# sahaRatul/sela

Measured on AMD Instinct MI355X. Metric: Msamples/s encode+decode, 16-bit stereo 44.1kHz, 1/2/4/8 GPU; bit-exact vs CPU, higher is better.
Workload: dtype f64+int64

## Files before the change

### sela_amd/csrc/sela_encode.hip

```cpp
#include <algorithm>
#include <atomic>
#include <random>
#include <vector>

#include "sela_device.h"

namespace sela {

constexpr int kPadC = 64;
constexpr int kHalfEntries = kBlock / 4;
constexpr int kParityLen = kPadC + kHalfEntries + 64;
constexpr int kLastT0 = (kHalfEntries + 64) / 32 - 1;
constexpr int kFirstT1 = (kHalfEntries - kPadC) / 32;
constexpr int kRingHalf = 64;
constexpr int kRingLen = 2 * kRingHalf + 64;
constexpr int kRingsPerXcd = 512;
constexpr int kXcds = 8;
constexpr int kPadS = 128;
constexpr int kSBufWords = (kPadS + kBlock) / 32 * 33;
constexpr int kSmallBase = 8992;
constexpr int kBigBytes = kSmallBase + 3008;
static_assert(kResWordsCap * 4 <= kSmallBase, "packed residue words must fit the dead sample buffer");
static_assert(kSBufWords * 4 <= kSmallBase && kSmallBase % 16 == 0, "sample buffer must end below the analysis arrays");
static_assert(kBigBytes >= 2 * kParityLen * 8, "the FP64 parity arrays must fit");

struct SmallArrays {
    double ac[104];
    double k[104];
    int64_t a[104];
    int32_t q[128];
};
static_assert(sizeof(SmallArrays) + kSmallBase <= kBigBytes, "analysis arrays overflow the LDS plan");

__device__ __forceinline__ void or_bits(uint32_t* buf, uint32_t pos, uint32_t v, uint32_t nbits)
{
    const uint32_t w = pos >> 5, sh = pos & 31;
    atomicOr(&buf[w], v << sh);
    if (sh + nbits > 32)
        atomicOr(&buf[w + 1], v >> (32 - sh));
}

__device__ __forceinline__ void or_bits_both(uint32_t* buf, uint32_t pos, uint32_t v)
{
    const uint64_t wide = (uint64_t)v << (pos & 31);
    uint32_t* const w = buf + (pos >> 5);
    atomicOr(w, (uint32_t)wide);
    atomicOr(w + 1, (uint32_t)(wide >> 32));
}

__device__ __attribute__((noinline)) uint32_t put_long_codeword(uint32_t* buf, uint32_t pos, uint32_t u, uint32_t k);

__device__ __forceinline__ uint32_t put_codeword(uint32_t* buf, uint32_t pos, uint32_t u, uint32_t k)
{
    uint32_t ones = u >> k;
    const uint32_t rem = k ? (__brev(u << (32 - k))) : 0u;
    while (ones >= 32) {
        or_bits(buf, pos, 0xFFFFFFFFu, 32);
        pos += 32;
        ones -= 32;
    }
    if (ones + 1 + k <= 32) {
        or_bits(buf, pos, ((1u << ones) - 1u) | (rem << (ones + 1)), ones + 1 + k);
        return pos + ones + 1 + k;
    }
    or_bits(buf, pos, (1u << ones) - 1u, ones + 1);
    pos += ones + 1;
    if (k) {
        or_bits(buf, pos, rem, k);
        pos += k;
    }
    return pos;
}

__device__ __attribute__((noinline)) uint32_t put_long_codeword(uint32_t* buf, uint32_t pos, uint32_t u, uint32_t k)
{
    return put_codeword(buf, pos, u, k);
}

template <int V>
__device__ __forceinline__ uint64_t rice_shifted_sum(const uint32_t (&u)[V], uint32_t k, bool small, uint32_t& lane_part)
{
    if (small) {
        uint32_t part = 0;
#pragma unroll
        for (int t = 0; t < V; t++)
            part += u[t] >> k;
        asm volatile("" : "+v"(part));
        lane_part = part;
        return wave_sum_small(part);
    }
    uint64_t part = 0;
#pragma unroll
    for (int t = 0; t < V; t++)
        part += u[t] >> k;
    lane_part = (uint32_t)part;
    return wave_sum_40(part);
}

template <int V>
__device__ __forceinline__ void rice_plan(const uint32_t (&u)[V], uint32_t n, uint32_t& best_k, uint64_t& best_bits, uint32_t& lane_or, uint32_t& lane_quotients)
{
    constexpr uint32_t kLast = SELA_MAX_RICE_PARAM - 1;
    lane_or = 0;
#pragma unroll
    for (int t = 0; t < V; t++)
        lane_or |= u[t];
    const bool small = !__any((lane_or >> 20) != 0);
    uint32_t p0, pa, pb, pc;
    const uint64_t t0 = rice_shifted_sum<V>(u, 0, small, p0);
    const uint64_t mean = n ? t0 / n : 0;
    uint32_t k = mean ? 63u - (uint32_t)__clzll(mean) : 0u;
    k = k > kLast - 1 ? kLast - 1 : k;
    uint64_t ta = t0;
    pa = p0;
    if (k)
        ta = rice_shifted_sum<V>(u, k, small, pa);
    uint64_t tb = rice_shifted_sum<V>(u, k + 1, small, pb);
    if (ta - tb <= n) {
        while (k > 0) {
            uint64_t tc = t0;
            pc = p0;
            if (k != 1)
                tc = rice_shifted_sum<V>(u, k - 1, small, pc);
            if (tc - ta > n)
                break;
            k--;
            tb = ta, pb = pa;
            ta = tc, pa = pc;
        }
    } else {
        for (;;) {
            k++;
            ta = tb, pa = pb;
            if (k == kLast)
                break;
            tb = rice_shifted_sum<V>(u, k + 1, small, pb);
            if (ta - tb <= n)
                break;
        }
    }
    best_k = k;
    best_bits = ta + (uint64_t)n * (1 + k);
    lane_quotients = pa;
}

__device__ __forceinline__ double scale_sample(int32_t s)
{
    constexpr double r = 1.0 / SELA_SAMPLE_SCALE;
    const double x = (double)s;
    const double q0 = x * r;
    const double e = __builtin_fma(-SELA_SAMPLE_SCALE, q0, x);
    return __builtin_fma(e, r, q0);
}

template <int kN>
__device__ __forceinline__ void unpack_stereo(uint32_t sig, const uint32_t (&w)[kN], int32_t (&raw)[kN])
{
    if (sig == 0) {
#pragma unroll
        for (int i = 0; i < kN; i++)
            raw[i] = (int32_t)(int16_t)(w[i] & 0xFFFFu);
    } else if (sig == 1) {
#pragma unroll
        for (int i = 0; i < kN; i++)
            raw[i] = (int32_t)w[i] >> 16;
    } else {
#pragma unroll
        for (int i = 0; i < kN; i++)
            raw[i] = (int32_t)(int16_t)(w[i] & 0xFFFFu) - ((int32_t)w[i] >> 16);
    }
}

typedef double f64x2 __attribute__((ext_vector_type(2)));
struct MeanFetch {
    f64x2 e0, e1, e2, e3, o0, o1, o2, o3;
};
#define SELA_MEAN_STR2(x) #x
#define SELA_MEAN_STR(x) SELA_MEAN_STR2(x)
#define SELA_MEAN_ISSUE(F, addr, OFF, sum)                                                    \
    asm volatile("ds_read_b128 %0, %9 offset:" #OFF "+0\n\t"                                    \
                 "ds_read_b128 %4, %9 offset:" #OFF "+5120\n\t"                                 \
                 "ds_read_b128 %1, %9 offset:" #OFF "+16\n\t"                                   \
                 "ds_read_b128 %5, %9 offset:" #OFF "+5136\n\t"                                 \
                 "ds_read_b128 %2, %9 offset:" #OFF "+32\n\t"                                   \
                 "ds_read_b128 %6, %9 offset:" #OFF "+5152\n\t"                                 \
                 "ds_read_b128 %3, %9 offset:" #OFF "+48\n\t"                                   \
                 "ds_read_b128 %7, %9 offset:" #OFF "+5168"                                      \
                 : "=&v"(F.e0), "=&v"(F.e1), "=&v"(F.e2), "=&v"(F.e3), "=&v"(F.o0), "=&v"(F.o1), "=&v"(F.o2), \
                 "=&v"(F.o3), "+v"(sum)                                                         \
                 : "v"(addr)                                                                    \
                 : "memory")
static_assert(kParityLen * 8 == 5120, "SELA_MEAN_ISSUE hard-codes the E -> O distance");

__device__ __forceinline__ void mean_wait(MeanFetch& f, double& sum)
{
    asm volatile("s_waitcnt lgkmcnt(0)"
                 : "+v"(f.e0), "+v"(f.e1), "+v"(f.e2), "+v"(f.e3), "+v"(f.o0), "+v"(f.o1), "+v"(f.o2), "+v"(f.o3), "+v"(sum));
}

__device__ __forceinline__ void mean_steps(const MeanFetch& f, double& sum)
{
    sum += f.e0[0]; sum += f.o0[0]; sum += f.e0[1]; sum += f.o0[1];
    sum += f.e1[0]; sum += f.o1[0]; sum += f.e1[1]; sum += f.o1[1];
    sum += f.e2[0]; sum += f.o2[0]; sum += f.e2[1]; sum += f.o2[1];
    sum += f.e3[0]; sum += f.o3[0]; sum += f.e3[1]; sum += f.o3[1];
}

typedef int sgpr16 __attribute__((ext_vector_type(16)));
typedef double f64x8 __attribute__((ext_vector_type(8)));

struct AcFetch {
    sgpr16 c_lo, c_hi;
    f64x2 o0, o1, o2, o3;
    f64x2 e0, e1, e2, e3;
};

#define SELA_AC_ISSUE_S(F, c_ptr, S0, S1, acc_e, acc_o)                                   \
    asm volatile("s_load_dwordx16 %0, %4, " #S0 "\n\ts_load_dwordx16 %1, %4, " #S1          \
                 : "=&s"(F.c_lo), "=&s"(F.c_hi), "+v"(acc_e), "+v"(acc_o) : "s"(c_ptr) : "memory")

#define SELA_AC_ISSUE_V(F, addr_e, addr_o, Q0, Q1, Q2, Q3, Q4, Q5, Q6, Q7, Q8, acc_e, acc_o) \
    asm volatile("ds_read2_b64 %0, %11 offset0:" #Q0 " offset1:" #Q1 "\n\t"                   \
                 "ds_read2_b64 %4, %10 offset0:" #Q1 " offset1:" #Q2 "\n\t"                   \
                 "ds_read2_b64 %1, %11 offset0:" #Q2 " offset1:" #Q3 "\n\t"                   \
                 "ds_read2_b64 %5, %10 offset0:" #Q3 " offset1:" #Q4 "\n\t"                   \
                 "ds_read2_b64 %2, %11 offset0:" #Q4 " offset1:" #Q5 "\n\t"                   \
                 "ds_read2_b64 %6, %10 offset0:" #Q5 " offset1:" #Q6 "\n\t"                   \
                 "ds_read2_b64 %3, %11 offset0:" #Q6 " offset1:" #Q7 "\n\t"                   \
                 "ds_read2_b64 %7, %10 offset0:" #Q7 " offset1:" #Q8                           \
                 : "=&v"(F.o0), "=&v"(F.o1), "=&v"(F.o2), "=&v"(F.o3), "=&v"(F.e0), "=&v"(F.e1), \
                 "=&v"(F.e2), "=&v"(F.e3), "+v"(acc_e), "+v"(acc_o)                           \
                 : "v"(addr_e), "v"(addr_o)                                                   \
                 : "memory")

__device__ __forceinline__ void ac_wait(AcFetch& f, double& acc_e, double& acc_o)
{
    asm volatile("s_waitcnt lgkmcnt(0)"
                 : "+s"(f.c_lo), "+s"(f.c_hi), "+v"(f.o0), "+v"(f.o1), "+v"(f.o2), "+v"(f.o3), "+v"(f.e0), "+v"(f.e1),
                 "+v"(f.e2), "+v"(f.e3), "+v"(acc_e), "+v"(acc_o));
}

__device__ __forceinline__ void ac_step(double cj, double nw, double& A, double& B, double& acc_e, double& acc_o)
{
    acc_e += cj * A;
    acc_o += cj * B;
    B = A;
    A = nw;
}

__device__ __forceinline__ void ac_steps_head(const AcFetch& f, double& A, double& B, double& acc_e, double& acc_o)
{
    const f64x8 c = __builtin_bit_cast(f64x8, f.c_lo);
    ac_step(c[0], f.o0[0], A, B, acc_e, acc_o);
    ac_step(c[1], f.e0[0], A, B, acc_e, acc_o);
}

__device__ __forceinline__ void ac_steps_tail(const AcFetch& f, double& A, double& B, double& acc_e, double& acc_o)
{
    const f64x8 c = __builtin_bit_cast(f64x8, f.c_lo), d = __builtin_bit_cast(f64x8, f.c_hi);
    ac_step(c[2], f.o0[1], A, B, acc_e, acc_o);
    ac_step(c[3], f.e0[1], A, B, acc_e, acc_o);
    ac_step(c[4], f.o1[0], A, B, acc_e, acc_o);
    ac_step(c[5], f.e1[0], A, B, acc_e, acc_o);
    ac_step(c[6], f.o1[1], A, B, acc_e, acc_o);
    ac_step(c[7], f.e1[1], A, B, acc_e, acc_o);
    ac_step(d[0], f.o2[0], A, B, acc_e, acc_o);
    ac_step(d[1], f.e2[0], A, B, acc_e, acc_o);
    ac_step(d[2], f.o2[1], A, B, acc_e, acc_o);
    ac_step(d[3], f.e2[1], A, B, acc_e, acc_o);
    ac_step(d[4], f.o3[0], A, B, acc_e, acc_o);
    ac_step(d[5], f.e3[0], A, B, acc_e, acc_o);
    ac_step(d[6], f.o3[1], A, B, acc_e, acc_o);
    ac_step(d[7], f.e3[1], A, B, acc_e, acc_o);
}

template <int JJ>
__device__ __forceinline__ void fir_taps_f64(int j0, int order, const int32_t* s_grp, const double* a_grp,
    double (&win)[kPerLane], double (&acc)[kPerLane])
{
    const int j = j0 + JJ + 1;
    if (j > order)
        return;
    const double aj = a_grp[JJ + 1];
    win[(32 - JJ - 1) & 31] = (double)s_grp[31 - JJ];
#pragma unroll
    for (int t = 0; t < kPerLane; t++)
        acc[t] = __builtin_fma(aj, win[(t - JJ - 1) & 31], acc[t]);
    __builtin_amdgcn_sched_barrier(0);
    if constexpr (JJ < 31)
        fir_taps_f64<JJ + 1>(j0, order, s_grp, a_grp, win, acc);
}
__device__ __forceinline__ const int32_t* fir_group_window(const int32_t* sT, int lane, int j0)
{
    const int e = kPadS + 32 * lane - j0 - 32;
    return sT + e + (e >> 5);
}
__device__ __forceinline__ const double* fir_group_coefs(const double* a_f, int j0)
{
    uint32_t at = (uint32_t)(uintptr_t)(const __attribute__((address_space(3))) double*)(a_f + j0);
    asm volatile("" : "+v"(at));
    return (const double*)(const __attribute__((address_space(3))) double*)(uintptr_t)at;
}

__device__ __attribute__((noinline)) void fir_plain(int order, int lane, const int32_t* sT, const int64_t* a, uint32_t* pred_out)
{
#pragma unroll 1
    for (int t = 0; t < kPerLane; t++) {
        uint64_t sum = (uint64_t)1 << (SELA_Q_SHIFT - 1);
#pragma unroll 1
        for (int j = 1; j <= order; j++) {
            const int e = kPadS + 32 * lane + t - j;
            sum += (uint64_t)a[j] * (uint64_t)(int64_t)sT[e + (e >> 5)];
        }
        pred_out[t * 64 + lane] = (uint32_t)(int32_t)((int64_t)sum >> SELA_Q_SHIFT);
    }
}

constexpr uint32_t kFuseSpinLimit = 1u << 18;
constexpr uint32_t kFuseNapLimit = 600000;
constexpr uint32_t kMeanWaitSpins = 24;

__device__ __forceinline__ void block_of(uint32_t e, uint32_t n_sig, uint32_t& frame, uint32_t& sig)
{
// ... 714 lines not shown
        asm volatile("s_waitcnt vmcnt(0)\n\ts_dcache_inv" ::: "memory");

        double A = E[-lane];
        double B = 0.0;
        uint32_t addr_e = (uint32_t)(uintptr_t)(__attribute__((address_space(3))) double*)(E - lane);
        uint32_t addr_o = (uint32_t)(uintptr_t)(__attribute__((address_space(3))) double*)(O - lane);
        const double* c_ptr = ring;
        AcFetch f0, f1;
        asm volatile("" : "+v"(A));
        SELA_AC_ISSUE_S(f0, c_ptr, 0, 64, acc_e, acc_o);
        SELA_AC_ISSUE_V(f0, addr_e, addr_o, 0, 1, 2, 3, 4, 5, 6, 7, 8, acc_e, acc_o);
        constexpr int kSwitch = kBlock / 2 / kRingHalf;
        const bool falling = !kFused && n_workers == 0 && fa.priorities != 0;
#pragma unroll 1
        for (int k = 0; k < kBlock / kRingHalf; k++) {
            if (falling && k == 0)
                __builtin_amdgcn_s_setprio(2);
            if (falling && k == kSwitch)
                __builtin_amdgcn_s_setprio(1);
            if (k == kSwitch) {
                wave_sync();
#pragma unroll
                for (int t = kFirstT1; t < kPerLane; t++)
                    mine1[half + 32 * t] = scale_sample(s[t]) - mean;
                wave_sync();
                addr_e -= kHalfEntries * 8;
                addr_o -= kHalfEntries * 8;
            }
            if (k >= 1 && k + 1 < kBlock / kRingHalf)
                store_chunk(k + 1, k >= kSwitch ? mine1 : mine);
#pragma unroll 1
            for (int it = 0; it < kRingHalf / 32; it++) {
                if (it == kRingHalf / 32 - 1)
                    asm volatile("s_waitcnt vmcnt(0)\n\ts_dcache_inv" ::: "memory");
                ac_wait(f0, acc_e, acc_o);
                SELA_AC_ISSUE_S(f1, c_ptr, 128, 192, acc_e, acc_o);
                ac_steps_head(f0, A, B, acc_e, acc_o);
                SELA_AC_ISSUE_V(f1, addr_e, addr_o, 8, 9, 10, 11, 12, 13, 14, 15, 16, acc_e, acc_o);
                ac_steps_tail(f0, A, B, acc_e, acc_o);
                ac_wait(f1, acc_e, acc_o);
                SELA_AC_ISSUE_S(f0, c_ptr, 256, 320, acc_e, acc_o);
                ac_steps_head(f1, A, B, acc_e, acc_o);
                SELA_AC_ISSUE_V(f0, addr_e, addr_o, 16, 17, 18, 19, 20, 21, 22, 23, 24, acc_e, acc_o);
                ac_steps_tail(f1, A, B, acc_e, acc_o);
                c_ptr += 32;
                addr_e += 128;
                addr_o += 128;
            }
            if (k & 1)
                c_ptr = ring;
        }
        ac_wait(f0, acc_e, acc_o);
        if (lane == 0)
            atomicExch(pool + slot, 0u);
    }
    wave_sync();

    SELA_STAMP(4);
    {
        const double ac0 = read_first_lane(acc_e);
        if (lane <= 50) {
            sm->ac[2 * lane] = lane == 0 ? 1.0 : acc_e / ac0;
            sm->ac[2 * lane + 1] = acc_o / ac0;
        }
    }
    wave_sync();

    double k_lo = 0.0, k_hi = 0.0;
    if (!kFused && n_workers == 0 && fa.priorities != 0)
        __builtin_amdgcn_s_setprio(1);
    else
        __builtin_amdgcn_s_setprio(2);
    {
        double g0a = sm->ac[lane + 1], g1a = g0a;
        double g0b = lane < 36 ? sm->ac[lane + 65] : 0.0, g1b = g0b;
        double err = 1.0;
        double g = read_first_lane(g1a);
        double ki = -g / err;
        err += g * ki;
        sm->k[0] = ki;
        constexpr int kTwoRegs = kMaxOrder - 64 + 1;
#pragma unroll 1
        for (int i = 1; i < kTwoRegs; i++) {
            const double sa = wave_shl1(read_first_lane(g1b), g1a);
            const double sb = wave_shl1_zero(g1b);
            g1a = sa + ki * g0a;
            g0a = sa * ki + g0a;
            g1b = sb + ki * g0b;
            g0b = sb * ki + g0b;
            g = read_first_lane(g1a);
            ki = -g / err;
            err += g * ki;
            sm->k[i] = ki;
        }
#pragma unroll 1
        for (int i = kTwoRegs; i < kMaxOrder; i++) {
            const double sa = wave_shl1_zero(g1a);
            g1a = sa + ki * g0a;
            g0a = sa * ki + g0a;
            g = read_first_lane(g1a);
            ki = -g / err;
            err += g * ki;
            sm->k[i] = ki;
        }
        wave_sync();
        k_lo = sm->k[lane];
        k_hi = lane < kMaxOrder - 64 ? sm->k[lane + 64] : 0.0;
        wave_sync();
    }
    if (kMode == 3) {
        uint64_t h_ac = hash_term(sm->ac[lane], lane) ^ (lane + 64 <= kMaxOrder ? hash_term(sm->ac[lane + 64], lane + 64) : 0ull);
        uint64_t h_k = hash_term(k_lo, lane) ^ (lane < kMaxOrder - 64 ? hash_term(k_hi, lane + 64) : 0ull);
        h_ac = lanes_xor<64>(h_ac);
        h_k = lanes_xor<64>(h_k);
        if (lane == 0) {
            uint64_t* const hp = reinterpret_cast<uint64_t*>(trace) + 2 * (size_t)block_id;
            hp[0] = h_ac;
            hp[1] = h_k;
        }
    }

    {
        constexpr bool kAcInLds = true;
        uint64_t* const sizes_pub = fa.sizes_pub;
        const uint64_t sizes_tag = fa.sizes_tag;
#define SELA_TAIL_TRACE_RESIDUES fa.trace_residues
#include "sela_encode_tail.inc"
#undef SELA_TAIL_TRACE_RESIDUES
    }
    SELA_STAMP(12);
    if (kFused) {
        const uint32_t g = frame / kGroupFrames;
        const uint32_t blocks_in_group = min((uint32_t)kGroupFrames, n_frames - g * kGroupFrames) * n_sig;
        stores_done();
        uint32_t last = 0;
        if (lane == 0)
            last = group_arrive(fa.group_count + (size_t)g * kGroupCountStride, fa.tag, blocks_in_group) ? 1u : 0u;
        if (__builtin_amdgcn_readfirstlane((int)last)) {
            drop_stale_lines();
            finish_group(fa, g, lane);
        }
    }
    SELA_STAMP(13);
    if (kMode == 2 && lane == 0)
        for (int i = 0; i < 13; i++)
            phase_cycles[(size_t)block_id * 16 + i] = (uint64_t)(stamp[i + 1] - stamp[i]);
}

constexpr int kTeamMirror = 24;
constexpr int kTeamWin = 16;
constexpr int kTeamAhead = 3;
constexpr int kTeamMeanChunk = 64;

template <int P>
struct TeamPlan {
    static constexpr int B = kWave / P;
    static constexpr int G = (kMaxOrder + 1 + P - 1) / P;
    static constexpr int kChunk = P == 8 ? 16 : 64;
    static constexpr int kRing = P == 8 ? 160 : 256;
    static constexpr int kStride = P == 8 ? kRing + kTeamMirror : kRing + 48;
    static constexpr int kPer = kChunk / P;
    static constexpr int kMeanPer = kTeamMeanChunk / P;
    static constexpr int kRingBytes = B * kStride * 8;
    static constexpr int kCwBase = kBigBytes;
    static constexpr int kKStride = 104;
    static constexpr int kQBase = kSmallBase;
    static constexpr int kQStride = 104;
    static constexpr int kSchurBase = B * kKStride;
    static constexpr int kSchurStride = P == 16 ? 2 * P * G : 0;
    static constexpr int kSchurBytes = P == 16 ? (kSchurBase + B * kSchurStride) * 8 : 0;
    static constexpr int kTailBytes = kCwBase + kCoefWordsCap * 4;
    static constexpr int kLdsBytes = kRingBytes > kTailBytes ? kRingBytes : kTailBytes;
    static_assert(kSchurBytes <= kLdsBytes, "the repack areas fit the kernel's LDS");
    static_assert(G + kTeamAhead <= kTeamWin && kChunk % kTeamWin == 0 && kRing % kChunk == 0 && kStride % 32 == (P == 8 ? 24 : 16) && kStride >= kRing + kTeamMirror, "team plan");
    static_assert((G * P - 1) + kChunk + kChunk <= kRing && 2 * kTeamMeanChunk <= kRing, "the ring must hold the lags' reach, the chunk in use and the chunk being written");
    static_assert(kLdsBytes * 12 <= 160 * 1024, "twelve waves per CU");
    static_assert(B * kKStride * 8 <= kQBase && B * kKStride * 8 <= kRingBytes && B * kQStride <= 104 * 8, "k[] in the dead rings below the q store; the q store inside SmallArrays::ac");
};

template <int P>
__device__ __forceinline__ uint32_t team_first(uint32_t v)
{
    if constexpr (P == 16) {
        return (uint32_t)__builtin_amdgcn_mov_dpp((int)v, 0x150 , 0xf, 0xf, true);
    } else {
        static_assert(P == 8, "teams of 8 or 16 lanes");
        const int q = __builtin_amdgcn_mov_dpp((int)v, 0x00 , 0xf, 0xf, true);
        return (uint32_t)__builtin_amdgcn_update_dpp(q, q, 0x114 , 0xf, 0xa , false);
    }
}
template <int P>
__device__ __forceinline__ double team_first(double v)
{
    const uint64_t x = __builtin_bit_cast(uint64_t, v);
    return __builtin_bit_cast(double, ((uint64_t)team_first<P>((uint32_t)(x >> 32)) << 32) | team_first<P>((uint32_t)x));
}

template <int kPer, int kStep>
__device__ __forceinline__ void team_load_raw(const int16_t* __restrict__ fp, uint32_t channels, uint32_t sig, int first, int32_t (&raw)[kPer])
{
    if (channels == 2) {
        const uint32_t* pw = reinterpret_cast<const uint32_t*>(fp) + first;
        uint32_t w[kPer];
        if constexpr (kStep == 1 && kPer % 4 == 0) {
#pragma unroll
            for (int u = 0; u < kPer / 4; u++) {
                const uint4 v = reinterpret_cast<const uint4*>(pw)[u];
                w[4 * u] = v.x, w[4 * u + 1] = v.y, w[4 * u + 2] = v.z, w[4 * u + 3] = v.w;
            }
        } else if constexpr (kStep == 1 && kPer % 2 == 0) {
#pragma unroll
            for (int u = 0; u < kPer / 2; u++) {
                const uint2 v = reinterpret_cast<const uint2*>(pw)[u];
                w[2 * u] = v.x, w[2 * u + 1] = v.y;
            }
        } else {
#pragma unroll
            for (int u = 0; u < kPer; u++)
                w[u] = pw[u * kStep];
        }
        if constexpr (kStep == 1) {
            const uint32_t first_shift = sig == 1 ? 16u : 0u;
            const uint32_t second_mask = sig == 2 ? 0xFFFFFFFFu : 0u;
#pragma unroll
            for (int i = 0; i < kPer; i++) {
                const int32_t a = (int32_t)(w[i] << (16 - first_shift)) >> 16, b = ((int32_t)w[i] >> 16) & (int32_t)second_mask;
                raw[i] = a - b;
            }
        } else {
            unpack_stereo<kPer>(sig, w, raw);
        }
    } else {
        const int16_t* const ps = fp + (size_t)first * channels + sig;
#pragma unroll
        for (int i = 0; i < kPer; i++)
            raw[i] = ps[(uint32_t)(i * kStep) * channels];
    }
}

template <int kPer, int kStep, bool kStereo>
__device__ __forceinline__ void team_fetch(const int16_t* __restrict__ fp, uint32_t channels, uint32_t sig, int first, uint32_t (&w)[kPer])
{
    if constexpr (kStereo) {
        const uint32_t* pw = reinterpret_cast<const uint32_t*>(fp) + first;
#pragma unroll
        for (int u = 0; u < kPer; u++)
            w[u] = pw[u * kStep];
    } else {
        const int16_t* const ps = fp + (size_t)first * channels + sig;
#pragma unroll
        for (int i = 0; i < kPer; i++)
            w[i] = (uint32_t)(int32_t)ps[(uint32_t)(i * kStep) * channels];
    }
}
template <int kPer, bool kStereo>
__device__ __forceinline__ void team_unpack(uint32_t sig, const uint32_t (&w)[kPer], int32_t (&raw)[kPer])
{
    if constexpr (kStereo) {
        unpack_stereo<kPer>(sig, w, raw);
    } else {
#pragma unroll
        for (int i = 0; i < kPer; i++)
            raw[i] = (int32_t)w[i];
    }
}

template <int kPer, int kStep, bool kCentre, bool kMirror, int kRing>
__device__ __forceinline__ void team_stage(double* ring_b, int pos, const int32_t (&raw)[kPer], double mean)
{
#pragma unroll
    for (int i = 0; i < kPer; i++) {
        const double x = scale_sample(raw[i]);
        const double c = kCentre ? x - mean : x;
        ring_b[pos + i * kStep] = c;
        if (kMirror && pos + i * kStep < kTeamMirror)
            ring_b[kRing + pos + i * kStep] = c;
    }
}

template <int kN>
__device__ __forceinline__ double team_chain(const double* x, double sum)
{
    constexpr int kBatch = 8;
    static_assert(kN % (2 * kBatch) == 0, "two batches per round");
    double u[kBatch], v[kBatch];
#pragma unroll
    for (int i = 0; i < kBatch; i++)
        u[i] = x[i];
#pragma unroll
    for (int i0 = 0; i0 < kN; i0 += 2 * kBatch) {
#pragma unroll
        for (int i = 0; i < kBatch; i++)
            v[i] = x[i0 + kBatch + i];
        __builtin_amdgcn_sched_barrier(0);
#pragma unroll
        for (int i = 0; i < kBatch; i++)
            sum += u[i];
        __builtin_amdgcn_sched_barrier(0);
        if (i0 + 2 * kBatch < kN) {
#pragma unroll
            for (int i = 0; i < kBatch; i++)
                u[i] = x[i0 + 2 * kBatch + i];
        }
        __builtin_amdgcn_sched_barrier(0);
#pragma unroll
        for (int i = 0; i < kBatch; i++)
// ... 63 lines not shown
                 : "v"(addr_w), "v"(addr_m), "n"(8 * (R0 + kTeamAhead)), "v"(acc[0]), "v"(acc[G - 1])
                 : "memory");
    asm volatile("s_waitcnt lgkmcnt(6)" : "+v"(W[R0 & (kTeamWin - 1)]), "+v"(M[R0 & 3]));
    const double m = M[R0 & 3];
    constexpr int kAheadOps = 5;
#pragma unroll
    for (int g0 = 0; g0 < G; g0 += kAheadOps) {
        double t[kAheadOps];
#pragma unroll
        for (int u = 0; u < kAheadOps; u++)
            if (g0 + u < G)
                t[u] = m * W[(R0 - g0 - u) & (kTeamWin - 1)];
#pragma unroll
        for (int u = 0; u < kAheadOps; u++)
            if (g0 + u < G)
                acc[g0 + u] += t[u];
    }
    __builtin_amdgcn_sched_barrier(0);
    if constexpr (R0 < kTeamWin - 1)
        team_ac_steps<G, R0 + 1>(W, M, acc, addr_w, addr_m);
}

template <int P>
struct TeamSchur {
    static constexpr int G = TeamPlan<P>::G;
    static constexpr bool kPhased = P == 16;
    static constexpr int kFirstStage(int g) { return g >= G || !kPhased ? 1 : kMaxOrder + 1 - P * g; }
    static constexpr int kEndStage(int g) { return g == 1 || !kPhased ? kMaxOrder : kFirstStage(g - 1); }
};

template <int P, int gFrom, int gTo>
__device__ __forceinline__ void team_schur_repack(double (&g0)[TeamPlan<P>::G], double (&g1)[TeamPlan<P>::G], double* __restrict__ area, int p)
{
    double* const w = area + gFrom * p;
    const double* const r = area + gTo * p;
#pragma unroll
    for (int c = 0; c < gFrom; c++) {
        w[c] = g0[c];
        w[P * gFrom + c] = g1[c];
    }
    wave_sync();
#pragma unroll
    for (int c = 0; c < gTo; c++) {
        g0[c] = r[c];
        g1[c] = r[P * gFrom + c];
    }
    wave_sync();
}

template <int P, int g>
__device__ __forceinline__ void team_schur_phases(double (&g0)[TeamPlan<P>::G], double (&g1)[TeamPlan<P>::G], double& ki, double& err,
    bool keeper, double* __restrict__ k_b, double* __restrict__ area, int p)
{
    using S = TeamSchur<P>;
    static_assert(S::kFirstStage(g) >= 1 && S::kFirstStage(g) < S::kEndStage(g) && P * g - 1 >= kMaxOrder - S::kFirstStage(g), "a phase starts when its last column is dead");
#pragma unroll 1
    for (int i = S::kFirstStage(g); i < S::kEndStage(g); i++) {
        const double crossing = wave_shl1_zero(g1[0]);
#pragma unroll
        for (int r = 0; r < g; r++) {
            const double sa = r + 1 < g ? g1[r + 1] : crossing;
            g1[r] = sa + ki * g0[r];
            g0[r] = sa * ki + g0[r];
        }
        const double first = team_first<P>(g1[0]);
        ki = -first / err;
        err += first * ki;
        if (keeper)
            k_b[i] = ki;
    }
    if constexpr (S::kPhased && g > 1) {
        team_schur_repack<P, g, g - 1>(g0, g1, area, p);
        team_schur_phases<P, g - 1>(g0, g1, ki, err, keeper, k_b, area, p);
    }
}

template <int kMode, int P>
__global__ __launch_bounds__(64) __attribute__((amdgpu_waves_per_eu(3, 3))) void k_encode_teams(
    const int16_t* __restrict__ pcm, uint32_t n_frames, uint32_t channels, uint32_t n_sig, BlockMeta* __restrict__ meta,
    uint32_t* __restrict__ slots, sela_hip_trace* __restrict__ trace, int force_plain_fir, uint64_t* __restrict__ phase_cycles,
    uint64_t* __restrict__ sizes_pub, uint64_t sizes_tag, uint32_t team_priorities)
{
    using Plan = TeamPlan<P>;
    constexpr int B = Plan::B, G = Plan::G, kPer = Plan::kPer, kMeanPer = Plan::kMeanPer, kChunk = Plan::kChunk, kRing = Plan::kRing;
    constexpr bool kTrace = kMode == 1;
    constexpr bool kFused = false;
    constexpr int kStep = P == 16 ? P : 1;
    __shared__ __attribute__((aligned(32))) unsigned char lds[Plan::kLdsBytes];
    unsigned char* const big = lds;
    uint32_t* const cw_buf = reinterpret_cast<uint32_t*>(lds + Plan::kCwBase);

    const int lane0 = threadIdx.x;
    const int b = lane0 / P, p = lane0 % P;
    const uint32_t wq = blockIdx.x % 8, wv = blockIdx.x / 8;
    const uint32_t sig = wv % n_sig;
    const uint32_t frame0 = ((wv / n_sig) * 8 + wq) * B;
    constexpr uint32_t frame_stride = 1;
    if (frame0 >= n_frames)
        return;
    const bool team_live = frame0 + (uint32_t)b * frame_stride < n_frames;
    const uint32_t my_frame = team_live ? frame0 + (uint32_t)b * frame_stride : frame0;
    const int16_t* const fp = pcm + (size_t)my_frame * kBlock * channels;
    double* const ring_b = reinterpret_cast<double*>(lds) + b * Plan::kStride;
    double* const k_b = reinterpret_cast<double*>(lds) + b * Plan::kKStride;
    long long wave_stamp[5];
    if (kMode == 2)
        wave_stamp[0] = clock64();

    double mean;
    if constexpr (P == 16) {
        static_assert(kStep == P, "lane p holds samples p, p + 16, .. of a chunk");
        set_wave_priority((int)(team_priorities & 0xFF));
        const double sum = channels == 2 ? team_row_mean_sum<kMeanPer, true>(fp, channels, sig, p) : team_row_mean_sum<kMeanPer, false>(fp, channels, sig, p);
        mean = sum / (double)kBlock;
    } else {
        constexpr int kChunks = kBlock / kTeamMeanChunk;
        const int mine = kStep == 1 ? p * kMeanPer : p;
        int32_t raw_a[kMeanPer], raw_b[kMeanPer];
        team_load_raw<kMeanPer, kStep>(fp, channels, sig, mine, raw_a);
        team_stage<kMeanPer, kStep, false, false, kRing>(ring_b, mine, raw_a, 0.0);
        team_load_raw<kMeanPer, kStep>(fp, channels, sig, kTeamMeanChunk + mine, raw_a);
        team_load_raw<kMeanPer, kStep>(fp, channels, sig, 2 * kTeamMeanChunk + mine, raw_b);
        double sum = 0.0;
        const uint32_t quarter_priorities = team_priorities;
        set_wave_priority((int)(quarter_priorities & 0xFF));
#pragma unroll 1
        for (int c = 0; c < kChunks; c++) {
            const int here = (c & 1) * kTeamMeanChunk, there = kTeamMeanChunk - here;
            if (c + 1 < kChunks)
                team_stage<kMeanPer, kStep, false, false, kRing>(ring_b, there + mine, raw_a, 0.0);
#pragma unroll
            for (int i = 0; i < kMeanPer; i++)
                raw_a[i] = raw_b[i];
            if (c + 3 < kChunks)
                team_load_raw<kMeanPer, kStep>(fp, channels, sig, (c + 3) * kTeamMeanChunk + mine, raw_b);
            wave_sync();
            sum = team_chain<kTeamMeanChunk>(ring_b + here, sum);
            wave_sync();
        }
        mean = sum / (double)kBlock;
    }
    if (kMode == 2)
        wave_stamp[1] = clock64();

    double acc[G];
    {
#pragma unroll
        for (int g = 0; g < G; g++)
            acc[g] = 0.0;
        for (int i = kChunk + p; i < Plan::kStride; i += P)
            ring_b[i] = 0.0;
        const int mine = kStep == 1 ? p * kPer : p;
        int32_t raw_a[kPer], raw_b[kPer];
        team_load_raw<kPer, kStep>(fp, channels, sig, mine, raw_a);
        team_stage<kPer, kStep, true, true, kRing>(ring_b, mine, raw_a, mean);
        team_load_raw<kPer, kStep>(fp, channels, sig, kChunk + mine, raw_a);
        team_load_raw<kPer, kStep>(fp, channels, sig, 2 * kChunk + mine, raw_b);
        wave_sync();
        const uint32_t ring_addr = (uint32_t)(uintptr_t)(__attribute__((address_space(3))) double*)ring_b;
        double W[kTeamWin], M[4];
#pragma unroll
        for (int i = 0; i < kTeamWin; i++)
            W[i] = 0.0;
        uint32_t idx_w = (uint32_t)((kRing - G * p) % kRing);
        uint32_t idx_m = 0, pos_stage = kChunk;
        uint32_t addr_w = ring_addr + 8 * idx_w, addr_m = ring_addr;
        asm volatile("ds_read_b64 %0, %6\n\tds_read_b64 %3, %7\n\t"
                     "ds_read_b64 %1, %6 offset:8\n\tds_read_b64 %4, %7 offset:8\n\t"
                     "ds_read_b64 %2, %6 offset:16\n\tds_read_b64 %5, %7 offset:16"
                     : "=&v"(W[0]), "=&v"(W[1]), "=&v"(W[2]), "=&v"(M[0]), "=&v"(M[1]), "=&v"(M[2])
                     : "v"(addr_w), "v"(addr_m)
                     : "memory");
        M[3] = 0.0;
        constexpr int kChunks = kBlock / kChunk;
        auto trips = [&]() {
#pragma unroll 1
            for (int it = 0; it < kChunk / kTeamWin; it++) {
                team_ac_steps<G, 0>(W, M, acc, addr_w, addr_m);
                idx_w += kTeamWin;
                idx_w = idx_w >= (uint32_t)kRing ? idx_w - kRing : idx_w;
                idx_m += kTeamWin;
                idx_m = idx_m >= (uint32_t)kRing ? idx_m - kRing : idx_m;
                addr_w = ring_addr + 8 * idx_w;
                addr_m = ring_addr + 8 * idx_m;
            }
        };
        auto stage_next = [&](const int32_t (&raw)[kPer]) {
            team_stage<kPer, kStep, true, true, kRing>(ring_b, (int)pos_stage + mine, raw, mean);
            pos_stage += kChunk;
            pos_stage = pos_stage >= (uint32_t)kRing ? 0u : pos_stage;
        };
        constexpr int kPrio2From = (int)(0.27 * kChunks), kPrio1From = (int)(0.71 * kChunks);
#pragma unroll 1
        for (int c = 0; c < kChunks; c++) {
            if (c == kPrio2From)
                set_wave_priority((int)((team_priorities >> 8) & 0xFF));
            if (c == kPrio1From)
                set_wave_priority((int)((team_priorities >> 16) & 0xFF));
            if (c + 1 < kChunks)
                stage_next(raw_a);
#pragma unroll
            for (int i = 0; i < kPer; i++)
                raw_a[i] = raw_b[i];
            if (c + 3 < kChunks)
                team_load_raw<kPer, kStep>(fp, channels, sig, (c + 3) * kChunk + mine, raw_b);
            trips();
        }
        asm volatile("s_waitcnt lgkmcnt(0)" : "+v"(W[0]), "+v"(W[1]), "+v"(W[2]), "+v"(M[0]), "+v"(M[1]), "+v"(M[2]));
    }
    wave_sync();
    if (kMode == 2)
        wave_stamp[2] = clock64();

    {
        const double ac0 = team_first<P>(acc[0]);
#pragma unroll
        for (int g = 0; g < G; g++)
            acc[g] = (p == 0 && g == 0) ? 1.0 : acc[g] / ac0;
    }
    if (kTrace && team_live) {
        sela_hip_trace* tr = trace + (size_t)my_frame * n_sig + sig;
        if (p == 0)
            tr->mean = mean;
#pragma unroll
        for (int g = 0; g < G; g++)
            if (G * p + g <= kMaxOrder)
                tr->ac[G * p + g] = acc[g];
    }
    if (kMode == 3) {
        uint64_t h = 0;
#pragma unroll
        for (int g = 0; g < G; g++)
            h ^= G * p + g <= kMaxOrder ? hash_term(acc[g], G * p + g) : 0ull;
        h = lanes_xor<P>(h);
        if (team_live && p == 0)
            reinterpret_cast<uint64_t*>(trace)[2 * ((size_t)my_frame * n_sig + sig)] = h;
    }

    {
        double g0[G], g1[G];
        const double next_first = wave_shl1_zero(acc[0]);
#pragma unroll
        for (int r = 0; r < G; r++) {
            const double v = r + 1 < G ? acc[r + 1] : next_first;
            g0[r] = g1[r] = (G * p + r < kMaxOrder) ? v : 0.0;
        }
        double err = 1.0;
        const bool keeper = p == 0;
        double g = team_first<P>(g1[0]);
        double ki = -g / err;
        err += g * ki;
        if (keeper)
            k_b[0] = ki;
        double* const area = reinterpret_cast<double*>(lds) + Plan::kSchurBase + b * Plan::kSchurStride;
        team_schur_phases<P, G>(g0, g1, ki, err, keeper, k_b, area, p);
    }
    wave_sync();
    if (kMode == 2)
        wave_stamp[3] = clock64();

    int8_t* const q_all = reinterpret_cast<int8_t*>(lds + Plan::kQBase);
#pragma unroll 1
    for (int bb = 0; bb < B; bb++) {
        const uint32_t frame = frame0 + (uint32_t)bb * frame_stride;
        if (frame >= n_frames)
            break;
        int lane_now = lane0;
        asm volatile("" : "+v"(lane_now));
        const int lane = lane_now;
        const double* const k_mine = reinterpret_cast<const double*>(lds) + bb * Plan::kKStride;
        const double k_lo = k_mine[lane];
        const double k_hi = lane < kMaxOrder - 64 ? k_mine[64 + lane] : 0.0;
        int order;
        {
            const unsigned long long b_lo = __ballot(fabs(k_lo) > SELA_ORDER_THRESHOLD);
            const unsigned long long b_hi = __ballot(lane < 36 && fabs(k_hi) > SELA_ORDER_THRESHOLD);
            order = b_hi ? 128 - __clzll(b_hi) : (b_lo ? 64 - __clzll(b_lo) : 1);
        }
        const double sqrt2 = SELA_SQRT2;
        double v_lo;
        if (lane == 0)
            v_lo = floor(64 * (-1 + (sqrt2 * sqrt(k_lo + 1))));
        else if (lane == 1)
            v_lo = floor(64 * (-1 + (sqrt2 * sqrt(-k_lo + 1))));
        else
            v_lo = floor(64 * k_lo);
        const double v_hi = floor(64 * k_hi);
        const int32_t q_lo = isnan(v_lo) ? 0 : (int32_t)v_lo;
        const int32_t q_hi = isnan(v_hi) ? 0 : (int32_t)v_hi;
        const bool wide = (lane < order && (q_lo < -128 || q_lo > 127)) || (lane + 64 < order && (q_hi < -128 || q_hi > 127));
        const bool escape = __any(wide);
        int8_t* const q_mine = q_all + bb * Plan::kQStride;
        q_mine[lane] = (int8_t)q_lo;
        if (lane < kMaxOrder - 64)
            q_mine[64 + lane] = (int8_t)q_hi;
        if (lane == 0) {
            q_mine[100] = (int8_t)order;
            q_mine[101] = escape ? 1 : 0;
        }
        if (escape) {
            int32_t* const q_wide = reinterpret_cast<int32_t*>(slots + ((size_t)frame * n_sig + sig) * kSlotWords);
            q_wide[lane] = q_lo;
            if (lane < kMaxOrder - 64)
                q_wide[64 + lane] = q_hi;
        }
        if (kTrace) {
            sela_hip_trace* tr = trace + (size_t)frame * n_sig + sig;
            tr->k[lane] = k_lo;
            if (lane < 36)
                tr->k[lane + 64] = k_hi;
        }
        if (kMode == 3) {
            uint64_t h = hash_term(k_lo, lane) ^ (lane < kMaxOrder - 64 ? hash_term(k_hi, lane + 64) : 0ull);
            h = lanes_xor<64>(h);
            if (lane == 0)
                reinterpret_cast<uint64_t*>(trace)[2 * ((size_t)frame * n_sig + sig) + 1] = h;
        }
    }
    wave_sync();

    SmallArrays* const sm = reinterpret_cast<SmallArrays*>(big + kSmallBase);
    long long stamp[14];
#pragma unroll 1
    for (int bb = 0; bb < B; bb++) {
        const uint32_t frame = frame0 + (uint32_t)bb * frame_stride;
        if (frame >= n_frames)
            break;
        int lane_now = lane0;
        asm volatile("" : "+v"(lane_now));
        const int lane = lane_now;
        const uint32_t block_id = frame * n_sig + sig;
        if (4 * (bb + 1) > B)
            set_wave_priority((int)((team_priorities >> 24) & 0xFF));
        const int8_t* const q_mine = q_all + bb * Plan::kQStride;
        const int order = (uint8_t)q_mine[100];
        int32_t q_lo = q_mine[lane], q_hi = lane < kMaxOrder - 64 ? q_mine[64 + lane] : 0;
        if (__builtin_amdgcn_readfirstlane((int)q_mine[101])) {
            const int32_t* const q_wide = reinterpret_cast<const int32_t*>(slots + (size_t)block_id * kSlotWords);
            q_lo = q_wide[lane];
            q_hi = lane < kMaxOrder - 64 ? q_wide[64 + lane] : 0;
        }
        const double mean = 0.0;
        int32_t s[kPerLane];
        {
            const int16_t* fb = pcm + (size_t)frame * kBlock * channels;
            if (channels == 2) {
                const uint32_t* fp2 = reinterpret_cast<const uint32_t*>(fb);
                uint32_t w[kPerLane];
#pragma unroll
                for (int t = 0; t < kPerLane; t++)
                    w[t] = fp2[lane + 64 * t];
                unpack_stereo<kPerLane>(sig, w, s);
            } else {
                const int16_t* const ps = fb + (size_t)lane * channels + sig;
#pragma unroll
                for (int t = 0; t < kPerLane; t++)
                    s[t] = ps[(uint32_t)(64 * t) * channels];
            }
        }
// ... 495 lines not shown
```

Before: 17350.

## Unroll P=16 team autocorrelation loop by ring revolution with dot2 stereo unpack

For the 16-lane team path, the chunk loop is unrolled four ways to match one ring revolution. This makes staging positions and mirror writes compile-time constants, drops the modulo index bookkeeping, and keeps raw packed words in registers instead of unpacked samples. Stereo unpacking becomes a single v_dot2_i32_i16 with a per-signal pick mask. Sample scaling replaces the two-FMA correction division with a two-term reciprocal expansion. These changes cut integer and VALU overhead in the hot loop, but they add code size, and the new scaling must stay bit-exact with the CPU division by 32767.

```diff
diff --git a/sela_amd/csrc/sela_encode.hip b/sela_amd/csrc/sela_encode.hip
--- a/sela_amd/csrc/sela_encode.hip
+++ b/sela_amd/csrc/sela_encode.hip
@@ -146,11 +146,11 @@
 
 __device__ __forceinline__ double scale_sample(int32_t s)
 {
-    constexpr double r = 1.0 / SELA_SAMPLE_SCALE;
+    constexpr double c1 = 0x1.00020004p-15, c2 = 0x1.0002000400080p-60;
+    static_assert(c1 == 1.0 / 32768 + 1.0 / (1 << 30) + 1.0 / (1ll << 45) && SELA_SAMPLE_SCALE == 32767.0, "the constants are those of a division by 32767");
     const double x = (double)s;
-    const double q0 = x * r;
-    const double e = __builtin_fma(-SELA_SAMPLE_SCALE, q0, x);
-    return __builtin_fma(e, r, q0);
+    const double q = x * c1;
+    return __builtin_fma(x, c2, q);
 }
 
 template <int kN>
@@ -169,6 +169,14 @@
         for (int i = 0; i < kN; i++)
             raw[i] = (int32_t)(int16_t)(w[i] & 0xFFFFu) - ((int32_t)w[i] >> 16);
     }
+}
+
+__device__ __forceinline__ uint32_t stereo_pick(uint32_t sig) { return sig == 0 ? 0x00000001u : sig == 1 ? 0x00010000u : 0xFFFF0001u; }
+__device__ __forceinline__ int32_t unpack_stereo_picked(uint32_t pick, uint32_t w)
+{
+    int32_t s;
+    asm("v_dot2_i32_i16 %0, %1, %2, 0" : "=v"(s) : "v"(w), "s"(pick));
+    return s;
 }
 
 typedef double f64x2 __attribute__((ext_vector_type(2)));
@@ -1189,6 +1197,9 @@
 constexpr int kTeamAhead = 3;
 constexpr int kTeamMeanChunk = 64;
 
+template <int I>
+struct IntConstant { static constexpr int value = I; };
+
 template <int P>
 struct TeamPlan {
     static constexpr int B = kWave / P;
@@ -1558,10 +1569,22 @@
             ring_b[i] = 0.0;
         const int mine = kStep == 1 ? p * kPer : p;
         int32_t raw_a[kPer], raw_b[kPer];
+        uint32_t w_a[kPer], w_b[kPer];
+        const bool stereo = channels == 2;
         team_load_raw<kPer, kStep>(fp, channels, sig, mine, raw_a);
         team_stage<kPer, kStep, true, true, kRing>(ring_b, mine, raw_a, mean);
-        team_load_raw<kPer, kStep>(fp, channels, sig, kChunk + mine, raw_a);
-        team_load_raw<kPer, kStep>(fp, channels, sig, 2 * kChunk + mine, raw_b);
+        if constexpr (P == 16) {
+            if (stereo) {
+                team_fetch<kPer, kStep, true>(fp, channels, sig, kChunk + mine, w_a);
+                team_fetch<kPer, kStep, true>(fp, channels, sig, 2 * kChunk + mine, w_b);
+            } else {
+                team_fetch<kPer, kStep, false>(fp, channels, sig, kChunk + mine, w_a);
+                team_fetch<kPer, kStep, false>(fp, channels, sig, 2 * kChunk + mine, w_b);
+            }
+        } else {
+            team_load_raw<kPer, kStep>(fp, channels, sig, kChunk + mine, raw_a);
+            team_load_raw<kPer, kStep>(fp, channels, sig, 2 * kChunk + mine, raw_b);
+        }
         wave_sync();
         const uint32_t ring_addr = (uint32_t)(uintptr_t)(__attribute__((address_space(3))) double*)ring_b;
         double W[kTeamWin], M[4];
@@ -1569,7 +1592,6 @@
         for (int i = 0; i < kTeamWin; i++)
             W[i] = 0.0;
         uint32_t idx_w = (uint32_t)((kRing - G * p) % kRing);
-        uint32_t idx_m = 0, pos_stage = kChunk;
         uint32_t addr_w = ring_addr + 8 * idx_w, addr_m = ring_addr;
         asm volatile("ds_read_b64 %0, %6\n\tds_read_b64 %3, %7\n\t"
                      "ds_read_b64 %1, %6 offset:8\n\tds_read_b64 %4, %7 offset:8\n\t"
@@ -1579,38 +1601,94 @@
                      : "memory");
         M[3] = 0.0;
         constexpr int kChunks = kBlock / kChunk;
-        auto trips = [&]() {
+        constexpr int kPrio2From = (int)(0.27 * kChunks), kPrio1From = (int)(0.71 * kChunks);
+        if constexpr (P == 16) {
+            static_assert(kRing == 4 * kChunk && kChunks % 4 == 0 && kStep == P && kPer * P == kChunk && (kRing & (kRing - 1)) == 0, "a revolution is four chunks; lane p stages samples p, p + 16, ..");
+            static_assert(kTeamMirror > P && kTeamMirror <= 2 * P, "the mirror takes sample 0 of every lane and sample 1 of the lanes below kTeamMirror - P");
+            static_assert(kPrio2From % 4 == 0 && kPrio1From % 4 == 2, "where the priority changes in the unrolled loop");
+            double* const stage_b = ring_b + p;
+            const bool in_mirror_twice = p < kTeamMirror - P;
+            const uint32_t* const wave_words = reinterpret_cast<const uint32_t*>(pcm) + (size_t)frame0 * kBlock;
+            const uint32_t lane_word = (my_frame - frame0) * (uint32_t)kBlock + (uint32_t)p;
+            const uint32_t pick = stereo ? stereo_pick(sig) : 0x00000001u;
+            uint32_t off_w = 8 * idx_w;
+            auto chunk_copy = [&](auto kc, int c, uint32_t (&w)[kPer]) {
+                constexpr int k = decltype(kc)::value;
+                constexpr int pos = (k + 1) % 4 * kChunk;
+                if (k != 3 || c + 1 < kChunks) {
+#pragma unroll
+                    for (int i = 0; i < kPer; i++) {
+                        const double x = scale_sample(unpack_stereo_picked(pick, w[i])) - mean;
+                        stage_b[pos + i * P] = x;
+                        if (pos == 0 && i == 0)
+                            stage_b[kRing] = x;
+                        if (pos == 0 && i == 1 && in_mirror_twice)
+                            stage_b[kRing + P] = x;
+                    }
+                }
+                const int ahead = min(c + 3, kChunks - 1);
+                if (stereo) {
+                    const uint32_t* const from = wave_words + ahead * kChunk;
+#pragma unroll
+                    for (int u = 0; u < kPer; u++)
+                        w[u] = from[lane_word + (uint32_t)(u * P)];
+                } else {
+                    team_fetch<kPer, kStep, false>(fp, channels, sig, ahead * kChunk + p, w);
+                }
 #pragma unroll 1
-            for (int it = 0; it < kChunk / kTeamWin; it++) {
-                team_ac_steps<G, 0>(W, M, acc, addr_w, addr_m);
-                idx_w += kTeamWin;
-                idx_w = idx_w >= (uint32_t)kRing ? idx_w - kRing : idx_w;
-                idx_m += kTeamWin;
-                idx_m = idx_m >= (uint32_t)kRing ? idx_m - kRing : idx_m;
-                addr_w = ring_addr + 8 * idx_w;
-                addr_m = ring_addr + 8 * idx_m;
+                for (int it = 0; it < kChunk / kTeamWin; it++) {
+                    team_ac_steps<G, 0>(W, M, acc, addr_w, addr_m);
+                    off_w = (off_w + 8 * kTeamWin) & (8 * kRing - 1);
+                    addr_w = ring_addr + off_w;
+                    addr_m += 8 * kTeamWin;
+                }
+            };
+#pragma unroll 1
+            for (int c = 0; c < kChunks; c += 4) {
+                if (c == kPrio2From)
+                    set_wave_priority((int)((team_priorities >> 8) & 0xFF));
+                addr_m = ring_addr;
+                chunk_copy(IntConstant<0>(), c, w_a);
+                chunk_copy(IntConstant<1>(), c + 1, w_b);
+                if (c + 2 == kPrio1From)
+                    set_wave_priority((int)((team_priorities >> 16) & 0xFF));
+                chunk_copy(IntConstant<2>(), c + 2, w_a);
+                chunk_copy(IntConstant<3>(), c + 3, w_b);
             }
-        };
-        auto stage_next = [&](const int32_t (&raw)[kPer]) {
-            team_stage<kPer, kStep, true, true, kRing>(ring_b, (int)pos_stage + mine, raw, mean);
-            pos_stage += kChunk;
-            pos_stage = pos_stage >= (uint32_t)kRing ? 0u : pos_stage;
-        };
-        constexpr int kPrio2From = (int)(0.27 * kChunks), kPrio1From = (int)(0.71 * kChunks);
+        } else {
+            uint32_t idx_m = 0, pos_stage = kChunk;
+            auto trips = [&]() {
 #pragma unroll 1
-        for (int c = 0; c < kChunks; c++) {
-            if (c == kPrio2From)
-                set_wave_priority((int)((team_priorities >> 8) & 0xFF));
-            if (c == kPrio1From)
-                set_wave_priority((int)((team_priorities >> 16) & 0xFF));
-            if (c + 1 < kChunks)
-                stage_next(raw_a);
-#pragma unroll
-            for (int i = 0; i < kPer; i++)
-                raw_a[i] = raw_b[i];
-            if (c + 3 < kChunks)
-                team_load_raw<kPer, kStep>(fp, channels, sig, (c + 3) * kChunk + mine, raw_b);
-            trips();
+                for (int it = 0; it < kChunk / kTeamWin; it++) {
+                    team_ac_steps<G, 0>(W, M, acc, addr_w, addr_m);
+                    idx_w += kTeamWin;
+                    idx_w = idx_w >= (uint32_t)kRing ? idx_w - kRing : idx_w;
+                    idx_m += kTeamWin;
+                    idx_m = idx_m >= (uint32_t)kRing ? idx_m - kRing : idx_m;
+                    addr_w = ring_addr + 8 * idx_w;
+                    addr_m = ring_addr + 8 * idx_m;
+                }
+            };
+            auto stage_next = [&](const int32_t (&raw)[kPer]) {
+                team_stage<kPer, kStep, true, true, kRing>(ring_b, (int)pos_stage + mine, raw, mean);
+                pos_stage += kChunk;
+                pos_stage = pos_stage >= (uint32_t)kRing ? 0u : pos_stage;
+            };
+#pragma unroll 1
+            for (int c = 0; c < kChunks; c++) {
+                if (c == kPrio2From)
+                    set_wave_priority((int)((team_priorities >> 8) & 0xFF));
+                if (c == kPrio1From)
+                    set_wave_priority((int)((team_priorities >> 16) & 0xFF));
+                if (c + 1 < kChunks)
+                    stage_next(raw_a);
+#pragma unroll
+                for (int i = 0; i < kPer; i++)
+                    raw_a[i] = raw_b[i];
+                if (c + 3 < kChunks)
+                    team_load_raw<kPer, kStep>(fp, channels, sig, (c + 3) * kChunk + mine, raw_b);
+                trips();
+            }
         }
         asm volatile("s_waitcnt lgkmcnt(0)" : "+v"(W[0]), "+v"(W[1]), "+v"(W[2]), "+v"(M[0]), "+v"(M[1]), "+v"(M[2]));
     }
```

Measured after the change: 17760, median of 6. +2.3%, better.
